# Li-Qingyun/RSCoTr

Measured on AMD Instinct MI355X. Metric: images/sec MTL train step (Swin-T 512^2, bs=2/GPU), higher is better.
Workload: dtype f32 (large products as three fp16 MFMAs on two-plane power-of-two-scaled splits of the fp32 operands, fp32 accumulate: fp32-FMA-class error; six bf16 MFMAs on three-plane splits where an operand has no range word)

## Files before the change

### rscotr_amd/csrc/gemm_group.hip

```cpp
#include "gemm_tiled_body.h"
#include "gemm_split_body.h"

namespace rscotr {
constexpr size_t GROUP_LDS_BYTES = 4 * (size_t)bf16x6_lds_words<128, 128, true, true, 0>();
template <int VAR>
__device__ __forceinline__ void gemm_group_dispatch(const int64_t* __restrict__ table, int n, const unsigned* __restrict__ amax_base) {
  extern __shared__ __attribute__((aligned(16))) float gemm_smem[];
  int lo = 0, hi = (n >> 3) - 1;
  while (lo < hi) {
    const int mid = (lo + hi + 1) >> 1;
    if ((int)table[(long)mid * 8 * 16 + 12] <= (int)blockIdx.x) lo = mid; else hi = mid - 1;
  }
  const int rel = (int)blockIdx.x - (int)table[(long)lo * 8 * 16 + 12];
  const int64_t* t = table + ((long)lo * 8 + (rel & 7)) * 16;
  const int jwg = rel >> 3;
  if (jwg >= (int)t[15]) return;
  GemmParams p;
  p.A = reinterpret_cast<const float*>(t[0]);
  p.B = reinterpret_cast<const float*>(t[1]);
  p.slabs = reinterpret_cast<float*>(t[2]);
  p.rs_slabs = reinterpret_cast<float*>(t[3]);
  p.kscale = reinterpret_cast<const float*>(t[4]);
  p.M = (int)t[5]; p.N = (int)t[6]; p.K = (int)t[7]; p.lda = (int)t[8]; p.ldb = (int)t[9];
  p.ksplit_len = (int)t[10]; p.splits = (int)t[11];
  p.krows_per = (int)t[13];
  p.C = nullptr; p.C2 = nullptr; p.bias = nullptr; p.aux = nullptr; p.pre = nullptr; p.resid = nullptr; p.rowscale = nullptr;
  p.ldc = p.N; p.act = ACT_NONE; p.accumulate = 0; p.rows_per = 1; p.rowsum_acc = 0;
  p.rowsum = p.rs_slabs;
  p.vecA = ((t[0] & 15) == 0) && (p.lda % 4 == 0);
  p.vecB = ((t[1] & 15) == 0) && (p.ldb % 4 == 0);
  p.vecC = 0;
  p.nb1 = 0; p.nb2 = 1;
  if constexpr (VAR == 7) {
    p.amax_a = amax_base + (unsigned)((uint64_t)t[14] >> 32) - 1;
    p.amax_b = amax_base + (unsigned)((uint64_t)t[14] & 0xffffffffu) - 1;
  }
  p.tiles = (VAR == 6 || VAR == 7) ? ((p.M + 127) / 128) * ((p.N + 127) / 128) : ((p.M + 63) / 64) * ((p.N + 63) / 64);
  const int tl_ = jwg % p.tiles, sl_ = jwg / p.tiles;
  const int q_ = p.tiles >> 3, r_ = p.tiles & 7, run_ = q_ + (r_ ? 1 : 0);
  int x_, pos_;
  if (tl_ < r_ * (q_ + 1)) { x_ = tl_ / (q_ + 1); pos_ = tl_ - x_ * (q_ + 1); }
  else { const int u_ = tl_ - r_ * (q_ + 1); x_ = r_ + u_ / q_; pos_ = u_ - (x_ - r_) * q_; }
  const int bx = 8 * (sl_ * run_ + pos_) + x_;
  const int gx = p.splits > 1 ? 8 * run_ * p.splits : p.tiles;
  if constexpr (VAR == 6) {
    gemm_bf16x6_body<128, 128, true, true, 0, true, true>(p, bx, gx, reinterpret_cast<unsigned*>(gemm_smem));
  } else if constexpr (VAR == 7) {
    gemm_bf16x6_body<128, 128, true, true, 0, true, true, true>(p, bx, gx, reinterpret_cast<unsigned*>(gemm_smem));
  } else {
    gemm_f32_body<64, 64, 2, 2, true, true, true, 1, true>(p, bx, gx, 0);
  }
}

template <int VAR>
__global__ __launch_bounds__(256) void gemm_f32_group_kernel(const int64_t* __restrict__ table, int n) {
  gemm_group_dispatch<VAR>(table, n, nullptr);
}
__global__ __launch_bounds__(256) __attribute__((amdgpu_waves_per_eu(2, 2))) void gemm_h3_group_kernel(
    const int64_t* __restrict__ table, int n, const unsigned* __restrict__ amax_base) {
  gemm_group_dispatch<7>(table, n, amax_base);
}
}
using namespace rscotr;

extern "C" int rscotr_gemm_dw_group(const int64_t* table, int n, int total_wgs, int variant, double flops,
                                    const uint32_t* amax_base, void* stream) {
  if (n < 0 || total_wgs < 0) return fail(RSCOTR_E_SHAPE, "rscotr_gemm_dw_group: negative count");
  if (n == 0 || total_wgs == 0) return RSCOTR_OK;
  if (!table) return fail(RSCOTR_E_ARG, "rscotr_gemm_dw_group: null table");
  ProfScope prof(PROF_GEMM, flops, (hipStream_t)stream, variant == 7 ? "rscotr::gemm_h3_group_kernel" : "rscotr::gemm_f32_group_kernel<%d>", variant);
  if (variant == 7) {
    if (!amax_base) return fail(RSCOTR_E_ARG, "rscotr_gemm_dw_group: variant 7 needs the value-range words (amax_base)");
    gemm_h3_group_kernel<<<dim3((unsigned)total_wgs), 256, GROUP_LDS_BYTES, (hipStream_t)stream>>>(table, n, amax_base);
  } else if (variant == 0) {
    gemm_f32_group_kernel<0><<<dim3((unsigned)total_wgs), 256, gemm_lds_bytes<64, 64, 1>(), (hipStream_t)stream>>>(table, n);
  } else if (variant == 6) {
    gemm_f32_group_kernel<6><<<dim3((unsigned)total_wgs), 256, GROUP_LDS_BYTES, (hipStream_t)stream>>>(table, n);
  } else {
    return fail(RSCOTR_E_ARG, "rscotr_gemm_dw_group: variant must be 0 (fp32 matrix pipe, 64 x 64 tiles, any problem), 6 (six-term bf16 split product, 128 x 128 tiles with edges) or 7 (fp16 split product on the same tiles)");
  }
  return check_launch("rscotr_gemm_dw_group");
}
```

### rscotr_amd/csrc/gemm_h3.hip

```cpp
#include "gemm_split_body.h"
#include "gemm_plan.h"

namespace rscotr {
template <int BM, int BN, bool AKM, bool BKM, int PIPE, bool EDGE = false, int OCC = 1, bool BPL = false>
__global__ __launch_bounds__(256, OCC) void gemm_h3_kernel(GemmParams p) {
  __shared__ __attribute__((aligned(16))) unsigned lds[bf16x6_lds_words<BM, BN, AKM, BKM, PIPE, true>()];
  gemm_bf16x6_body<BM, BN, AKM, BKM, PIPE, false, EDGE, true, BPL>(p, blockIdx.x, gridDim.x, lds);
}
template <bool AKM, bool BKM, bool EDGE = false, bool ONESET = false>
__global__ __launch_bounds__(256) __attribute__((amdgpu_waves_per_eu(2, 2))) void gemm_h3_128_kernel(GemmParams p) {
  __shared__ __attribute__((aligned(16))) unsigned lds[bf16x6_lds_words<128, 128, AKM, BKM, 0, true>()];
  gemm_bf16x6_body<128, 128, AKM, BKM, 0, false, EDGE, true, false, ONESET>(p, blockIdx.x, gridDim.x, lds);
}

void launch_h3(const GemmParams& p, const GemmPlan& pl, hipStream_t s) {
  if (pl.b_from_planes) {
    gemm_h3_kernel<64, 64, false, false, 2, false, 4, true><<<dim3(pl.nwg), 256, 0, s>>>(p);
    return;
  }
  with_split_cfg(pl, [&](auto bm, auto pipe, auto edge) {
    with_layout(pl.a_kmajor, pl.b_kmajor, [&](auto ak, auto bk) {
      constexpr int BM = decltype(bm)::value, PIPE = decltype(pipe)::value;
      constexpr bool EDGE = decltype(edge)::value, AK = decltype(ak)::value, BK = decltype(bk)::value;
      if constexpr (BM == 128) {
        if (AK && BK && (p.lda >= (1 << 26) || p.ldb >= (1 << 26))) gemm_h3_128_kernel<AK, BK, EDGE, AK && BK><<<dim3(pl.nwg), 256, 0, s>>>(p);
        else gemm_h3_128_kernel<AK, BK, EDGE><<<dim3(pl.nwg), 256, 0, s>>>(p);
      } else if (PIPE == 2 && !EDGE && !AK) {
        gemm_h3_kernel<64, 64, false, BK, 2, false, 4><<<dim3(pl.nwg), 256, 0, s>>>(p);
      } else {
        gemm_h3_kernel<BM, BM, AK, BK, PIPE, EDGE><<<dim3(pl.nwg), 256, 0, s>>>(p);
      }
    });
  });
}
}
```

### rscotr_amd/csrc/gemm_split_body.h

```cpp
#pragma once
#include "gemm_common.h"
#include <type_traits>

namespace rscotr {
typedef __bf16 bf16x2_t __attribute__((ext_vector_type(2)));
template <int NPL>
__device__ __forceinline__ void split_pair(float a, float b, unsigned (&out)[3]) {
  const f32x2_t x = {a, b};
  const bf16x2_t h = __builtin_convertvector(x, bf16x2_t);
  out[0] = __builtin_bit_cast(unsigned, h);
  const f32x2_t r1 = x - __builtin_convertvector(h, f32x2_t);
  const bf16x2_t m = __builtin_convertvector(r1, bf16x2_t);
  out[1] = __builtin_bit_cast(unsigned, m);
  if (NPL == 3) {
    const f32x2_t r2 = r1 - __builtin_convertvector(m, f32x2_t);
    out[2] = __builtin_bit_cast(unsigned, __builtin_convertvector(r2, bf16x2_t));
  } else {
    out[2] = 0u;
  }
}

__device__ __forceinline__ unsigned cvt_pk_bf16(float lo, float hi) {
  const f32x2_t x = {lo, hi};
  return __builtin_bit_cast(unsigned, __builtin_convertvector(x, bf16x2_t));
}

template <int NPL>
__device__ __forceinline__ void split_rows4(const float4& e, const float4& o, uint4 (&out)[3]) {
  f32x2_t e01 = {e.x, e.y}, e23 = {e.z, e.w}, o01 = {o.x, o.y}, o23 = {o.z, o.w};
#pragma unroll
  for (int pl = 0; pl < NPL; ++pl) {
    const unsigned h0 = cvt_pk_bf16(e01.x, o01.x), h1 = cvt_pk_bf16(e01.y, o01.y);
    const unsigned h2 = cvt_pk_bf16(e23.x, o23.x), h3 = cvt_pk_bf16(e23.y, o23.y);
    out[pl] = make_uint4(h0, h1, h2, h3);
    if (pl + 1 < NPL) {
      const f32x2_t fe01 = {__uint_as_float(h0 << 16), __uint_as_float(h1 << 16)};
      const f32x2_t fe23 = {__uint_as_float(h2 << 16), __uint_as_float(h3 << 16)};
      const f32x2_t fo01 = {__uint_as_float(h0 & 0xffff0000u), __uint_as_float(h1 & 0xffff0000u)};
      const f32x2_t fo23 = {__uint_as_float(h2 & 0xffff0000u), __uint_as_float(h3 & 0xffff0000u)};
      e01 -= fe01; e23 -= fe23; o01 -= fo01; o23 -= fo23;
    }
  }
}

__device__ __forceinline__ void split_rows4_h(const float4& e, const float4& o, const H3Scale& k, uint4 (&out)[3]) {
  unsigned a[3], b[3], c[3], d[3];
  split_pair_h(e.x, o.x, k, a);
  split_pair_h(e.y, o.y, k, b);
  split_pair_h(e.z, o.z, k, c);
  split_pair_h(e.w, o.w, k, d);
  out[0] = make_uint4(a[0], b[0], c[0], d[0]);
  out[1] = make_uint4(a[1], b[1], c[1], d[1]);
}

template <int R, bool KM, int NPL, int SBK = 16, bool H16 = false>
struct SplitOperand {
  static_assert(!H16 || NPL == 2, "the fp16 split has two planes");
  static constexpr int LDR = SBK * NPL + 8;
  static constexpr int KP = SBK / 2;
  static constexpr int Q = SBK / 4;
  static constexpr int WORDS = KM ? NPL * KP * R : R * LDR / 2;
  static constexpr int ITEMS = KM ? KP * R / 4 : R * Q;
  static constexpr int NV = (ITEMS + 255) / 256;
  float4 v[NV], w[NV];

  template <bool EDGE = false>
  __device__ __forceinline__ void load(const float* __restrict__ P, int ld, int row0, int k0, int tid, int rlast = 0, int klim = 0) {
#pragma unroll
    for (int i = 0; i < NV; ++i) {
      const int idx = tid + i * 256;
      if (ITEMS % 256 == 0 || idx < ITEMS) {
        if (!KM) {
          const int row = EDGE ? min(row0 + idx / Q, rlast) : row0 + idx / Q;
          const int kk = k0 + (idx % Q) * 4;
          v[i] = *reinterpret_cast<const float4*>(P + (long)row * ld + (EDGE ? min(kk, klim - 4) : kk));
          if (EDGE && kk >= klim) v[i] = make_float4(0.f, 0.f, 0.f, 0.f);
        } else {
          const int kp = idx / (R / 4), r4 = (idx % (R / 4)) * 4;
          const int ka = k0 + 2 * kp, col = EDGE ? min(row0 + r4, rlast) : row0 + r4;
          if (!EDGE) {
            const float* src = P + (long)ka * ld + col;
            v[i] = *reinterpret_cast<const float4*>(src);
            w[i] = *reinterpret_cast<const float4*>(src + ld);
          } else {
            v[i] = *reinterpret_cast<const float4*>(P + (long)min(ka, klim - 1) * ld + col);
            w[i] = *reinterpret_cast<const float4*>(P + (long)min(ka + 1, klim - 1) * ld + col);
            if (ka >= klim) v[i] = make_float4(0.f, 0.f, 0.f, 0.f);
            if (ka + 1 >= klim) w[i] = make_float4(0.f, 0.f, 0.f, 0.f);
          }
        }
      }
    }
  }
  __device__ __forceinline__ unsigned thread_offset(int ld, int row0, int tid, bool edge, int rlast) const {
    static_assert(!KM || ITEMS % 256 == 0, "whole items per thread");
    const int col = row0 + (tid % (R / 4)) * 4;
    return 4u * (unsigned)(2 * (tid / (R / 4)) * ld + (edge ? min(col, rlast) : col));
  }
  static __device__ __forceinline__ float4 load_row(const float* P, int ld, int krow, int klim, unsigned off) {
    typedef unsigned vec4u __attribute__((ext_vector_type(4)));
    const long left = 4l * ld * max(klim - krow, 0);
    const __amdgpu_buffer_rsrc_t d = __builtin_amdgcn_make_buffer_rsrc(const_cast<float*>(P + (long)krow * ld), 0,
                                                                        (int)(unsigned)min(left, 0xffffffffl), 0x00020000);
    const vec4u t = __builtin_amdgcn_raw_buffer_load_b128(d, (int)off, 0, 0);
    return make_float4(__uint_as_float(t.x), __uint_as_float(t.y), __uint_as_float(t.z), __uint_as_float(t.w));
  }
  __device__ __forceinline__ void load_rows(const float* __restrict__ P, int ld, int k0, int klim, unsigned off) {
#pragma unroll
    for (int i = 0; i < NV; ++i) {
      const int krow = k0 + i * (2 * 256 / (R / 4));
      v[i] = load_row(P, ld, krow, klim, off);
      w[i] = load_row(P, ld, krow + 1, klim, off);
    }
  }
  __device__ __forceinline__ void scale_k(const float* __restrict__ ks, int per, int k0, int tid, int klast = 0x7ffffffe) {
#pragma unroll
    for (int i = 0; i < NV; ++i) {
      const int idx = tid + i * 256;
      if (ITEMS % 256 == 0 || idx < ITEMS) {
        const int k = k0 + 2 * (idx / (R / 4));
        const float f0 = ks[min(k, klast) / per], f1 = ks[min(k + 1, klast) / per];
        v[i].x *= f0; v[i].y *= f0; v[i].z *= f0; v[i].w *= f0;
        w[i].x *= f1; w[i].y *= f1; w[i].z *= f1; w[i].w *= f1;
      }
    }
  }
  __device__ __forceinline__ void scale_k_fetch(const float* __restrict__ ks, int per, int k0, int wave, int klast, float (&f)[4 * NV]) const {
    static_assert(!KM || R == 128, "two k pairs per wavefront");
#pragma unroll
    for (int i = 0; i < NV; ++i) {
      const int kb = k0 + 4 * wave + i * (2 * 256 / (R / 4));
      int k = min(kb, klast), q = k / per, r = k - q * per;
#pragma unroll
      for (int j = 0; j < 4; ++j) {
        const int kn = min(kb + j, klast);
        if (kn != k) {
          k = kn;
          if (++r == per) { r = 0; ++q; }
        }
        f[4 * i + j] = *(const __attribute__((address_space(4))) float*)(ks + q);
      }
    }
  }
  __device__ __forceinline__ void scale_k_apply(const float (&f)[4 * NV], int tid) {
    const bool hi = (tid / (R / 4)) & 1;
#pragma unroll
    for (int i = 0; i < NV; ++i) {
      const float f0 = hi ? f[4 * i + 2] : f[4 * i], f1 = hi ? f[4 * i + 3] : f[4 * i + 1];
      v[i].x *= f0; v[i].y *= f0; v[i].z *= f0; v[i].w *= f0;
      w[i].x *= f1; w[i].y *= f1; w[i].z *= f1; w[i].w *= f1;
    }
  }
  __device__ __forceinline__ void accum(float4& a, int tid, float f = 1.f) const {
    static_assert(!KM || 256 % (R / 4) == 0, "row sums assume one row group per thread");
#pragma unroll
    for (int i = 0; i < NV; ++i)
      if (ITEMS % 256 == 0 || tid + i * 256 < ITEMS) {
        a.x = fmaf(f, v[i].x + w[i].x, a.x); a.y = fmaf(f, v[i].y + w[i].y, a.y);
        a.z = fmaf(f, v[i].z + w[i].z, a.z); a.w = fmaf(f, v[i].w + w[i].w, a.w);
      }
  }
  __device__ __forceinline__ void store(unsigned* S, int tid, const H3Scale& hs = H3Scale{1.f, 2048.f}) const {
#pragma unroll
    for (int i = 0; i < NV; ++i) {
      const int idx = tid + i * 256;
      if (ITEMS % 256 == 0 || idx < ITEMS) {
        if (!KM) {
          const int row = idx / Q, kq = (idx % Q) * 4;
          unsigned ab[3], cd[3];
          if constexpr (H16) {
            split_pair_h(v[i].x, v[i].y, hs, ab);
            split_pair_h(v[i].z, v[i].w, hs, cd);
          } else {
            split_pair<NPL>(v[i].x, v[i].y, ab);
            split_pair<NPL>(v[i].z, v[i].w, cd);
          }
          unsigned* dst = S + (row * LDR + kq) / 2;
#pragma unroll
          for (int pl = 0; pl < NPL; ++pl) {
            uint2 q;
            q.x = ab[pl];
            q.y = cd[pl];
            *reinterpret_cast<uint2*>(dst + pl * (SBK / 2)) = q;
          }
        } else {
          const int kp = idx / (R / 4), r4 = (idx % (R / 4)) * 4;
          uint4 q[3];
          if constexpr (H16) split_rows4_h(v[i], w[i], hs, q);
          else split_rows4<NPL>(v[i], w[i], q);
#pragma unroll
          for (int pl = 0; pl < NPL; ++pl) *reinterpret_cast<uint4*>(S + (pl * KP + kp) * R + r4) = q[pl];
        }
      }
    }
  }
  static __device__ __forceinline__ void frag(const unsigned* S, int row, int g, int ks, bf16x8 (&f)[3]) {
    if (!KM) {
      const unsigned* q = S + (row * LDR + 16 * ks + 8 * g) / 2;
#pragma unroll
      for (int pl = 0; pl < NPL; ++pl) f[pl] = __builtin_bit_cast(bf16x8, *reinterpret_cast<const uint4*>(q + pl * (SBK / 2)));
    } else {
#pragma unroll
      for (int pl = 0; pl < NPL; ++pl) {
        const unsigned* q = S + (pl * KP + 8 * ks + 4 * g) * R + row;
        uint4 t;
        t.x = q[0]; t.y = q[R]; t.z = q[2 * R]; t.w = q[3 * R];
        f[pl] = __builtin_bit_cast(bf16x8, t);
      }
    }
  }
};

template <int R, int SBK>
struct PlaneOperandH {
  using Lay = SplitOperand<R, false, 2, SBK, true>;
  static_assert(R == 64 && SBK == 32, "one 32-byte piece per thread");
  static constexpr int WORDS = Lay::WORDS, KP = Lay::KP;
  typedef float vec4 __attribute__((ext_vector_type(4)));
  vec4 v0, v1;
  template <bool EDGE = false>
  __device__ __forceinline__ void load(const float* __restrict__ P, int ld, int row0, int k0, int tid, int = 0, int = 0) {
    const vec4* src = reinterpret_cast<const vec4*>(P) + ((long)(k0 / SBK) * ld + row0) * 8 + tid * 2;
    v0 = src[0];
    v1 = src[1];
  }
  __device__ __forceinline__ void store(unsigned* S, int tid, const H3Scale& = H3Scale{1.f, 2048.f}) const {
    vec4* dst = reinterpret_cast<vec4*>(S + (tid >> 2) * (Lay::LDR / 2) + (tid & 3) * 8);
    dst[0] = v0;
    dst[1] = v1;
  }
  static __device__ __forceinline__ void frag(const unsigned* S, int row, int g, int ks, bf16x8 (&f)[3]) { Lay::frag(S, row, g, ks, f); }
};

__device__ const float bf16x6_one = 1.f;
template <int PIPE> constexpr int bf16x6_bk() { return PIPE == 2 ? 32 : PIPE == 0 ? X6_BK0 : 16; }
constexpr int X6_D2 = 2, H3_VPM = 8, H3_DPM = 2;
template <int PIPE> constexpr int bf16x6_depth() { return PIPE == 2 ? X6_D2 : 1; }
template <int BM, int BN, bool AKM, bool BKM, int PIPE, bool EDGE, bool H16>
constexpr bool h3_two_tiles() { return H16 && PIPE == 0 && BM == 128 && BN == 128 && AKM && BKM; }

template <int BM, int BN, bool AKM, bool BKM, int PIPE, bool H16 = false>
constexpr int bf16x6_lds_words() {
  constexpr int NPL = H16 ? 2 : 3;
  return (PIPE ? 2 : 1) * (SplitOperand<BM, AKM, NPL, bf16x6_bk<PIPE>(), H16>::WORDS + SplitOperand<BN, BKM, NPL, bf16x6_bk<PIPE>(), H16>::WORDS);
}

template <int BM, int BN, bool AKM, bool BKM, int PIPE, bool SLAB, bool EDGE = false, bool H16 = false, bool BPL = false, bool ONESET = false>
__device__ __forceinline__ void gemm_bf16x6_body(GemmParams& p, const int bx, const int gx, unsigned* lds) {
  constexpr bool TWO = !ONESET && h3_two_tiles<BM, BN, AKM, BKM, PIPE, EDGE, H16>();
  constexpr int NPL = H16 ? 2 : 3, SBK = bf16x6_bk<PIPE>(), D = TWO ? 2 : bf16x6_depth<PIPE>();
  constexpr int MT = BM / 64, NT = BN / 64;
  using OA = SplitOperand<BM, AKM, NPL, SBK, H16>;
  static_assert(!BPL || (H16 && !BKM && !EDGE && PIPE == 2), "B from planes: the interior pipelined fp16 kernel");
  using OB = typename std::conditional<BPL, PlaneOperandH<BN, SBK>, SplitOperand<BN, BKM, NPL, SBK, H16>>::type;
  H3Scale ha{1.f, 2048.f}, hb{1.f, 2048.f};
  float inva = 1.f, invb = 1.f;
  unsigned ra = 0u, rb = 0u;
  if constexpr (H16) {
    ra = p.amax_a[(long)(threadIdx.x & (kAmaxPlanes - 1)) * kAmaxStride];
    rb = p.amax_b[(long)(threadIdx.x & (kAmaxPlanes - 1)) * kAmaxStride];
  }
  auto h3_scales = [&]() {
    if constexpr (H16) {
      if constexpr (TWO) {
        int ln = (int)__lane_id();
        asm volatile("" : "+v"(ln));
        ra = amax_fold_lane(ra, ln); rb = amax_fold_lane(rb, ln);
      } else {
        ra = amax_fold(ra); rb = amax_fold(rb);
      }
      const int ea = h3_scale_exp(ra), eb = h3_scale_exp(rb);
      ha.sc = __uint_as_float((unsigned)ea << 23); ha.sc2 = __uint_as_float((unsigned)(ea + 11) << 23);
      hb.sc = __uint_as_float((unsigned)eb << 23); hb.sc2 = __uint_as_float((unsigned)(eb + 11) << 23);
      inva = __uint_as_float((unsigned)(254 - ea) << 23); invb = __uint_as_float((unsigned)(254 - eb) << 23);
    }
  };
  constexpr int NBUF = PIPE ? 2 : 1;
  unsigned* sA[2] = {lds, lds + (NBUF - 1) * OA::WORDS};
  unsigned* sB[2] = {lds + NBUF * OA::WORDS, lds + NBUF * OA::WORDS + (NBUF - 1) * OB::WORDS};
  int tid = threadIdx.x, lane = tid & 63, wave = tid >> 6;
  int wm = wave >> 1, wn = wave & 1;
  const int tiles_n = EDGE ? (p.N + BN - 1) / BN : p.N / BN;
  const int alast = EDGE ? (AKM ? p.M - 4 : p.M - 1) : 0, blast = EDGE ? (BKM ? p.N - 4 : p.N - 1) : 0;
  int tile, split = 0;
  if (p.splits == 1) {
    tile = xcd_swizzle(bx, gx);
  } else {
    const int x = bx & 7, j = bx >> 3;
    const int q = p.tiles >> 3, r = p.tiles & 7, run = q + (r ? 1 : 0);
    const int nt = q + (x < r ? 1 : 0);
    split = j / run;
    const int tl = j - split * run;
    if (tl >= nt) return;
    tile = (x < r ? x * (q + 1) : r * (q + 1) + (x - r) * q) + tl;
  }
  const int m0 = (tile / tiles_n) * BM, n0 = (tile % tiles_n) * BN;
  const int kbeg = split * p.ksplit_len;
  const int kend = min(p.K, kbeg + p.ksplit_len);
  const int nk = EDGE ? (kend - kbeg + SBK - 1) / SBK : (kend - kbeg) / SBK;
  const int klast = EDGE ? p.K - 1 : 0x7ffffffe;

  f32x16 acc[MT][NT];
  f32x16 acc2[H16 ? MT : 1][H16 ? NT : 1];
#pragma unroll
  for (int i = 0; i < MT; ++i)
#pragma unroll
    for (int j = 0; j < NT; ++j)
#pragma unroll
      for (int r = 0; r < 16; ++r) {
        acc[i][j][r] = 0.f;
        if constexpr (H16) acc2[i][j][r] = 0.f;
      }
  OA las[D];
  OB lbs[D];
  OA& la = las[0];
  OB& lb = lbs[0];
  const bool do_rs = AKM && p.rowsum && n0 == 0;
  float4 rs = make_float4(0.f, 0.f, 0.f, 0.f);
  int fr = lane & 31, g = lane >> 5;
  auto fetch = [&](int t) {
    la.template load<EDGE>(p.A, p.lda, m0, kbeg + t * SBK, tid, alast, p.K);
    lb.template load<EDGE>(p.B, p.ldb, n0, kbeg + t * SBK, tid, blast, p.K);
    if (AKM && p.kscale) la.scale_k(p.kscale, p.krows_per, kbeg + t * SBK, tid, klast);
  };
  auto stage = [&](unsigned* a_s, unsigned* b_s) {
    if (AKM && do_rs) la.accum(rs, tid);
    la.store(a_s, tid, ha);
    lb.store(b_s, tid, hb);
  };
  auto mma = [&](const unsigned* a_s, const unsigned* b_s) {
    int ra0 = wm * (BM / 2) + fr, rb0 = wn * (BN / 2) + fr;
    if constexpr (TWO) asm volatile("" : "+v"(ra0), "+v"(rb0));
#pragma unroll
    for (int ks = 0; ks < SBK / 16; ++ks) {
      bf16x8 af[MT][3], bf[NT][3];
#pragma unroll
      for (int i = 0; i < MT; ++i) OA::frag(a_s, ra0 + i * 32, g, ks, af[i]);
#pragma unroll
      for (int j = 0; j < NT; ++j) OB::frag(b_s, rb0 + j * 32, g, ks, bf[j]);
      if constexpr (H16) {
#pragma unroll
        for (int tm = 0; tm < 3; ++tm)
#pragma unroll
          for (int i = 0; i < MT; ++i)
#pragma unroll
            for (int j = 0; j < NT; ++j) {
              const f16x8 a = __builtin_bit_cast(f16x8, af[i][tm == 0 ? 1 : 0]), b = __builtin_bit_cast(f16x8, bf[j][tm == 1 ? 1 : 0]);
              if (tm < 2) acc2[i][j] = __builtin_amdgcn_mfma_f32_32x32x16_f16(a, b, acc2[i][j], 0, 0, 0);
              else acc[i][j] = __builtin_amdgcn_mfma_f32_32x32x16_f16(a, b, acc[i][j], 0, 0, 0);
            }
        continue;
      }
      constexpr int PA[6] = {2, 0, 1, 1, 0, 0}, PB[6] = {0, 2, 1, 0, 1, 0};
#pragma unroll
      for (int tm = 0; tm < 6; ++tm)
#pragma unroll
        for (int i = 0; i < MT; ++i)
#pragma unroll
          for (int j = 0; j < NT; ++j)
            acc[i][j] = __builtin_amdgcn_mfma_f32_32x32x16_bf16(af[i][PA[tm]], bf[j][PB[tm]], acc[i][j], 0, 0, 0);
    }
  };
  if (PIPE == 2) {
    constexpr int U = (D % 2 == 0) ? D : 2 * D;
    constexpr int NMFMA = MT * NT * (H16 ? 3 : 6) * (SBK / 16);
    constexpr int VPM = H16 ? H3_VPM : 4, DPM = H16 ? H3_DPM : 1;
    const float* ksp = (AKM && p.kscale) ? p.kscale : &bf16x6_one;
    const int ksper = (AKM && p.kscale) ? p.krows_per : 0x7fffffff;
#pragma unroll
    for (int d = 0; d < D; ++d) {
      const int tt = min(d, nk - 1);
      las[d].template load<EDGE>(p.A, p.lda, m0, kbeg + tt * SBK, tid, alast, p.K);
      lbs[d].template load<EDGE>(p.B, p.ldb, n0, kbeg + tt * SBK, tid, blast, p.K);
    }
    h3_scales();
    if (AKM) las[0].scale_k(ksp, ksper, kbeg, tid, klast);
    if (AKM) las[0].accum(rs, tid);
    las[0].store(sA[0], tid, ha);
    lbs[0].store(sB[0], tid, hb);
    __syncthreads();
    for (int t0 = 0; t0 < nk; t0 += U) {
#pragma unroll
      for (int s = 0; s < U; ++s) {
        const int t = t0 + s;
        if (t < nk) {
          {
            const int tt = min(t + D, nk - 1);
            las[s % D].template load<EDGE>(p.A, p.lda, m0, kbeg + tt * SBK, tid, alast, p.K);
            lbs[s % D].template load<EDGE>(p.B, p.ldb, n0, kbeg + tt * SBK, tid, blast, p.K);
          }
          mma(sA[s & 1], sB[s & 1]);
          if (AKM) las[(s + 1) % D].scale_k(ksp, ksper, kbeg + min(t + 1, nk - 1) * SBK, tid, klast);
          if (AKM) las[(s + 1) % D].accum(rs, tid, t + 1 < nk ? 1.f : 0.f);
          las[(s + 1) % D].store(sA[(s + 1) & 1], tid, ha);
          lbs[(s + 1) % D].store(sB[(s + 1) & 1], tid, hb);
#pragma unroll
          for (int i = 0; i < NMFMA; ++i) {
            __builtin_amdgcn_sched_group_barrier(0x008, 1, 0);
            __builtin_amdgcn_sched_group_barrier(0x002, VPM, 0);
            __builtin_amdgcn_sched_group_barrier(0x200, DPM, 0);
          }
          __syncthreads();
        }
      }
    }
  } else if (PIPE) {
    fetch(0);
    h3_scales();
    stage(sA[0], sB[0]);
    if (nk > 1) fetch(1);
    __syncthreads();
    for (int t = 0; t < nk; ++t) {
      const bool odd = t & 1;
      mma(odd ? sA[1] : sA[0], odd ? sB[1] : sB[0]);
      if (t + 1 < nk) {
        stage(odd ? sA[0] : sA[1], odd ? sB[0] : sB[1]);
        if (t + 2 < nk) fetch(t + 2);
      }
      __syncthreads();
    }
  } else if constexpr (TWO) {
    float kf[4 * OA::NV];
    const unsigned offa = la.thread_offset(p.lda, m0, tid, EDGE, alast);
    const unsigned offb = lb.thread_offset(p.ldb, n0, tid, EDGE, blast);
    const int wave_u = __builtin_amdgcn_readfirstlane(tid >> 6);
    auto factors = [&](int t) {
      if (p.kscale) la.scale_k_fetch(p.kscale, p.krows_per, kbeg + t * SBK, wave_u, klast, kf);
    };
    auto fetch2 = [&](auto set, int t) {
      constexpr int S = decltype(set)::value;
      const int k0 = __builtin_amdgcn_readfirstlane(kbeg + t * SBK);
      las[S].load_rows(p.A, p.lda, k0, kend, offa);
      lbs[S].load_rows(p.B, p.ldb, k0, kend, offb);
    };
    auto stage2 = [&](auto set) {
      constexpr int S = decltype(set)::value;
#pragma unroll
      for (int i = 0; i < OA::NV; ++i) {
        asm volatile("" : "+v"(las[S].v[i].x), "+v"(las[S].v[i].y), "+v"(las[S].v[i].z), "+v"(las[S].v[i].w));
        asm volatile("" : "+v"(las[S].w[i].x), "+v"(las[S].w[i].y), "+v"(las[S].w[i].z), "+v"(las[S].w[i].w));
        asm volatile("" : "+v"(lbs[S].v[i].x), "+v"(lbs[S].v[i].y), "+v"(lbs[S].v[i].z), "+v"(lbs[S].v[i].w));
        asm volatile("" : "+v"(lbs[S].w[i].x), "+v"(lbs[S].w[i].y), "+v"(lbs[S].w[i].z), "+v"(lbs[S].w[i].w));
      }
      if (p.kscale) las[S].scale_k_apply(kf, tid);
      if (do_rs) las[S].accum(rs, tid);
      las[S].store(sA[0], tid, ha);
      lbs[S].store(sB[0], tid, hb);
    };
    constexpr std::integral_constant<int, 0> s0{};
    constexpr std::integral_constant<int, 1> s1{};
    factors(0);
    fetch2(s0, 0);
    fetch2(s1, 1);
    h3_scales();
    for (int t = 0; t < nk; t += 2) {
      __syncthreads();
      stage2(s0);
      if (t + 1 < nk) factors(t + 1);
      fetch2(s0, t + 2);
      __syncthreads();
      mma(sA[0], sB[0]);
      if (t + 1 < nk) {
        __syncthreads();
        stage2(s1);
        if (t + 2 < nk) factors(t + 2);
        fetch2(s1, t + 3);
        __syncthreads();
        mma(sA[0], sB[0]);
      }
    }
  } else {
    fetch(0);
    h3_scales();
    for (int t = 0; t < nk; ++t) {
      __syncthreads();
      stage(sA[0], sB[0]);
      if (t + 1 < nk) fetch(t + 1);
      __syncthreads();
      mma(sA[0], sB[0]);
    }
  }

  if constexpr (TWO) {
    asm volatile("" : "+v"(tid));
    lane = tid & 63; wave = tid >> 6; wm = wave >> 1; wn = wave & 1; fr = lane & 31; g = lane >> 5;
  }
  if (AKM && do_rs) {
    __syncthreads();
    constexpr int KL = 256 / (BM / 4) < OA::KP ? 256 / (BM / 4) : OA::KP;
    float4* red = reinterpret_cast<float4*>(lds);
    if (tid < KL * BM / 4) red[tid] = rs;
    __syncthreads();
    if (tid < BM) {
      const float* rf = reinterpret_cast<const float*>(lds);
      float v = 0.f;
#pragma unroll
      for (int k = 0; k < KL; ++k) v += rf[k * BM + tid];
      const int m = m0 + tid;
      if (!EDGE || m < p.M) {
        if (p.splits > 1 || SLAB) p.rs_slabs[(long)split * p.M + m] = v;
        else p.rowsum[m] = p.rowsum_acc ? p.rowsum[m] + v : v;
      }
    }
  }

  if constexpr (H16) {
#pragma unroll
    for (int i = 0; i < MT; ++i)
#pragma unroll
      for (int j = 0; j < NT; ++j)
#pragma unroll
        for (int r = 0; r < 16; ++r) acc[i][j][r] = fmaf(acc2[i][j][r], 0x1p-11f, acc[i][j][r]) * inva * invb;
  }
  if (p.splits > 1 || SLAB) {
    float* slab = p.slabs + (long)split * p.M * p.N;
#pragma unroll
    for (int i = 0; i < MT; ++i)
#pragma unroll
      for (int j = 0; j < NT; ++j) {
        const int n = n0 + wn * (BN / 2) + j * 32 + fr;
#pragma unroll
        for (int r = 0; r < 16; ++r) {
          const int m = m0 + wm * (BM / 2) + i * 32 + (r & 3) + 8 * (r >> 2) + 4 * g;
          if (!EDGE || (m < p.M && n < p.N)) slab[(long)m * p.N + n] = acc[i][j][r];
        }
      }
    return;
  }
  if constexpr (BM == 128 && BN == 128 && !EDGE) {
    if (p.act == ACT_RELU_BITS || p.act == ACT_RELU_GRAD_BITS) {
      const bool fwd = p.act == ACT_RELU_BITS;
      const long widx = ((long)(m0 / 128) * (p.N / 128) + n0 / 128) * 256 + tid;
      unsigned long long bits = fwd ? 0ull : reinterpret_cast<const unsigned long long*>(p.aux)[widx];
      float amx = 0.f;
#pragma unroll
      for (int i = 0; i < MT; ++i)
#pragma unroll
        for (int j = 0; j < NT; ++j) {
          const int n = n0 + wn * (BN / 2) + j * 32 + fr;
          const float bv = p.bias ? p.bias[n] : 0.f;
          float* crow = p.C + (long)(m0 + wm * (BM / 2) + i * 32 + 4 * g) * p.ldc + n;
#pragma unroll
          for (int r = 0; r < 16; ++r) {
            const int b = (i * NT + j) * 16 + r;
            float v = acc[i][j][r] + bv;
            if (fwd) {
              v = fmaxf(v, 0.f);
              bits |= (unsigned long long)(v > 0.f) << b;
            } else {
              v = ((bits >> b) & 1ull) ? v : 0.f;
            }
            crow[(long)((r & 3) + 8 * (r >> 2)) * p.ldc] = v;
            amx = fmaxf(amx, fabsf(v));
          }
        }
      if (fwd) reinterpret_cast<unsigned long long*>(p.pre)[widx] = bits;
      amax_commit(p.amax_out, amx);
      return;
    }
  }
  const bool plain = !p.pre && p.act == ACT_NONE && !p.resid && !p.accumulate && !p.rowscale && !p.C2;
  const bool one_extra = BM == 64 && !p.C2 &&
                         ((p.act == ACT_RELU_GRAD || p.act == ACT_GELU_GRAD) ? 1 : 0) + (p.resid ? 1 : 0) + (p.accumulate ? 1 : 0) == 1;
  const bool noload = !plain && (p.act == ACT_NONE || p.act == ACT_RELU || p.act == ACT_GELU) && !p.resid && !p.accumulate &&
                      !p.rowscale && !p.C2;
  float amx = 0.f;
#pragma unroll
  for (int i = 0; i < MT; ++i)
#pragma unroll
    for (int j = 0; j < NT; ++j) {
      const int n = n0 + wn * (BN / 2) + j * 32 + fr;
      if (EDGE && n >= p.N) continue;
      const float bv = p.bias ? p.bias[n] : 0.f;
      const int mb = m0 + wm * (BM / 2) + i * 32 + 4 * g;
      float* crow = p.C + (long)mb * p.ldc + n;
      if (one_extra) {
        epilogue_tile16<EDGE>(p, acc[i][j], bv, mb, n, amx);
        __builtin_amdgcn_sched_barrier(0);
      } else if (noload) {
        epilogue_noload16<EDGE>(p, acc[i][j], bv, mb, n, amx);
      } else if (plain) {
#pragma unroll
        for (int r = 0; r < 16; ++r)
          if (!EDGE || mb + (r & 3) + 8 * (r >> 2) < p.M) {
            const float v = acc[i][j][r] + bv;
            crow[(long)((r & 3) + 8 * (r >> 2)) * p.ldc] = v;
            amx = fmaxf(amx, fabsf(v));
          }
      } else {
#pragma unroll
        for (int g4 = 0; g4 < 4; ++g4) {
          float v[4];
#pragma unroll
          for (int u = 0; u < 4; ++u) v[u] = acc[i][j][4 * g4 + u] + bv;
          epilogue_rows4<EDGE>(p, v, mb + 8 * g4, n, amx);
          __builtin_amdgcn_sched_barrier(0);
        }
      }
    }
  amax_commit(p.amax_out, amx);
}
}
```

Before: 216.1.

## Double-buffer LDS in two-set fp16 split GEMM slab path to drop a barrier per step

Adds a second LDS stage for the two-register-set h3 split-product GEMM when it writes split-K slabs (the grouped dW kernel). Staging the next K tile into the other LDS buffer while the current one feeds the MFMAs removes one __syncthreads per K step and lets the stores overlap the matrix work. The cost is double the LDS footprint for the grouped kernel, which needs a raised dynamic shared-memory attribute and may lower occupancy.

```diff
diff --git a/rscotr_amd/csrc/gemm_group.hip b/rscotr_amd/csrc/gemm_group.hip
--- a/rscotr_amd/csrc/gemm_group.hip
+++ b/rscotr_amd/csrc/gemm_group.hip
@@ -3,6 +3,7 @@
 
 namespace rscotr {
 constexpr size_t GROUP_LDS_BYTES = 4 * (size_t)bf16x6_lds_words<128, 128, true, true, 0>();
+constexpr size_t GROUP_H3_LDS_BYTES = 4 * (size_t)bf16x6_lds_words<128, 128, true, true, 0, true, h3_two_stages<true, true>()>();
 template <int VAR>
 __device__ __forceinline__ void gemm_group_dispatch(const int64_t* __restrict__ table, int n, const unsigned* __restrict__ amax_base) {
   extern __shared__ __attribute__((aligned(16))) float gemm_smem[];
@@ -71,7 +72,12 @@
   ProfScope prof(PROF_GEMM, flops, (hipStream_t)stream, variant == 7 ? "rscotr::gemm_h3_group_kernel" : "rscotr::gemm_f32_group_kernel<%d>", variant);
   if (variant == 7) {
     if (!amax_base) return fail(RSCOTR_E_ARG, "rscotr_gemm_dw_group: variant 7 needs the value-range words (amax_base)");
-    gemm_h3_group_kernel<<<dim3((unsigned)total_wgs), 256, GROUP_LDS_BYTES, (hipStream_t)stream>>>(table, n, amax_base);
+    if constexpr (GROUP_H3_LDS_BYTES > 48 * 1024) {
+      static const hipError_t raised = hipFuncSetAttribute(reinterpret_cast<const void*>(gemm_h3_group_kernel),
+                                                           hipFuncAttributeMaxDynamicSharedMemorySize, (int)GROUP_H3_LDS_BYTES);
+      (void)raised;
+    }
+    gemm_h3_group_kernel<<<dim3((unsigned)total_wgs), 256, GROUP_H3_LDS_BYTES, (hipStream_t)stream>>>(table, n, amax_base);
   } else if (variant == 0) {
     gemm_f32_group_kernel<0><<<dim3((unsigned)total_wgs), 256, gemm_lds_bytes<64, 64, 1>(), (hipStream_t)stream>>>(table, n);
   } else if (variant == 6) {
diff --git a/rscotr_amd/csrc/gemm_h3.hip b/rscotr_amd/csrc/gemm_h3.hip
--- a/rscotr_amd/csrc/gemm_h3.hip
+++ b/rscotr_amd/csrc/gemm_h3.hip
@@ -9,7 +9,8 @@
 }
 template <bool AKM, bool BKM, bool EDGE = false, bool ONESET = false>
 __global__ __launch_bounds__(256) __attribute__((amdgpu_waves_per_eu(2, 2))) void gemm_h3_128_kernel(GemmParams p) {
-  __shared__ __attribute__((aligned(16))) unsigned lds[bf16x6_lds_words<128, 128, AKM, BKM, 0, true>()];
+  constexpr bool STG2 = !ONESET && h3_two_tiles<128, 128, AKM, BKM, 0, EDGE, true>() && h3_two_stages<false, EDGE>();
+  __shared__ __attribute__((aligned(16))) unsigned lds[bf16x6_lds_words<128, 128, AKM, BKM, 0, true, STG2>()];
   gemm_bf16x6_body<128, 128, AKM, BKM, 0, false, EDGE, true, false, ONESET>(p, blockIdx.x, gridDim.x, lds);
 }
 
diff --git a/rscotr_amd/csrc/gemm_split_body.h b/rscotr_amd/csrc/gemm_split_body.h
--- a/rscotr_amd/csrc/gemm_split_body.h
+++ b/rscotr_amd/csrc/gemm_split_body.h
@@ -239,10 +239,12 @@
 template <int BM, int BN, bool AKM, bool BKM, int PIPE, bool EDGE, bool H16>
 constexpr bool h3_two_tiles() { return H16 && PIPE == 0 && BM == 128 && BN == 128 && AKM && BKM; }
 
-template <int BM, int BN, bool AKM, bool BKM, int PIPE, bool H16 = false>
+template <bool SLAB, bool EDGE>
+constexpr bool h3_two_stages() { return SLAB; }
+template <int BM, int BN, bool AKM, bool BKM, int PIPE, bool H16 = false, bool STG2 = false>
 constexpr int bf16x6_lds_words() {
   constexpr int NPL = H16 ? 2 : 3;
-  return (PIPE ? 2 : 1) * (SplitOperand<BM, AKM, NPL, bf16x6_bk<PIPE>(), H16>::WORDS + SplitOperand<BN, BKM, NPL, bf16x6_bk<PIPE>(), H16>::WORDS);
+  return (PIPE || STG2 ? 2 : 1) * (SplitOperand<BM, AKM, NPL, bf16x6_bk<PIPE>(), H16>::WORDS + SplitOperand<BN, BKM, NPL, bf16x6_bk<PIPE>(), H16>::WORDS);
 }
 
 template <int BM, int BN, bool AKM, bool BKM, int PIPE, bool SLAB, bool EDGE = false, bool H16 = false, bool BPL = false, bool ONESET = false>
@@ -275,7 +277,8 @@
       inva = __uint_as_float((unsigned)(254 - ea) << 23); invb = __uint_as_float((unsigned)(254 - eb) << 23);
     }
   };
-  constexpr int NBUF = PIPE ? 2 : 1;
+  constexpr bool STG2 = TWO && h3_two_stages<SLAB, EDGE>();
+  constexpr int NBUF = (PIPE || STG2) ? 2 : 1;
   unsigned* sA[2] = {lds, lds + (NBUF - 1) * OA::WORDS};
   unsigned* sB[2] = {lds + NBUF * OA::WORDS, lds + NBUF * OA::WORDS + (NBUF - 1) * OB::WORDS};
   int tid = threadIdx.x, lane = tid & 63, wave = tid >> 6;
@@ -433,8 +436,8 @@
       las[S].load_rows(p.A, p.lda, k0, kend, offa);
       lbs[S].load_rows(p.B, p.ldb, k0, kend, offb);
     };
-    auto stage2 = [&](auto set) {
-      constexpr int S = decltype(set)::value;
+    auto stage2 = [&](auto set, auto stg) {
+      constexpr int S = decltype(set)::value, G = decltype(stg)::value;
 #pragma unroll
       for (int i = 0; i < OA::NV; ++i) {
         asm volatile("" : "+v"(las[S].v[i].x), "+v"(las[S].v[i].y), "+v"(las[S].v[i].z), "+v"(las[S].v[i].w));
@@ -444,30 +447,56 @@
       }
       if (p.kscale) las[S].scale_k_apply(kf, tid);
       if (do_rs) las[S].accum(rs, tid);
-      las[S].store(sA[0], tid, ha);
-      lbs[S].store(sB[0], tid, hb);
+      las[S].store(sA[G], tid, ha);
+      lbs[S].store(sB[G], tid, hb);
     };
     constexpr std::integral_constant<int, 0> s0{};
     constexpr std::integral_constant<int, 1> s1{};
+    if constexpr (STG2) {
+      factors(0);
+      fetch2(s0, 0);
+      fetch2(s1, 1);
+      h3_scales();
+      stage2(s0, s0);
+      if (1 < nk) factors(1);
+      int t = 0;
+      for (; t + 1 < nk; t += 2) {
+        fetch2(s0, t + 2);
+        __syncthreads();
+        mma(sA[0], sB[0]);
+        stage2(s1, s1);
+        if (t + 2 < nk) factors(t + 2);
+        fetch2(s1, t + 3);
+        __syncthreads();
+        mma(sA[1], sB[1]);
+        stage2(s0, s0);
+        if (t + 3 < nk) factors(t + 3);
+      }
+      if (t < nk) {
+        __syncthreads();
+        mma(sA[0], sB[0]);
+      }
+    } else {
     factors(0);
     fetch2(s0, 0);
     fetch2(s1, 1);
     h3_scales();
     for (int t = 0; t < nk; t += 2) {
       __syncthreads();
-      stage2(s0);
+      stage2(s0, s0);
       if (t + 1 < nk) factors(t + 1);
       fetch2(s0, t + 2);
       __syncthreads();
       mma(sA[0], sB[0]);
       if (t + 1 < nk) {
         __syncthreads();
-        stage2(s1);
+        stage2(s1, s0);
         if (t + 2 < nk) factors(t + 2);
         fetch2(s1, t + 3);
         __syncthreads();
         mma(sA[0], sB[0]);
       }
+    }
     }
   } else {
     fetch(0);
```

New measurement: 216.8, median of 6. Within noise of the previous version (+0.3%).
